# wgurecky/bipymc

Measured on AMD Instinct MI355X. Metric: chain-updates/sec, higher is better.
Workload: dtype f64

## Files before the change

bipymc_amd/csrc/kernels.h:

```cpp
#pragma once
#ifndef __HIPCC_RTC__
#include <hip/hip_runtime.h>
#include <stdint.h>
#endif

#include "philox.h"

#ifdef BPM_STAMPS
#define BPM_STAMP(i)                                                                          \
    do {                                                                                      \
        __builtin_amdgcn_sched_barrier(0);                                                    \
        unsigned long long _t;                                                                \
        asm volatile("s_memtime %0\n\ts_waitcnt lgkmcnt(0)" : "=s"(_t)::"memory");            \
        __builtin_amdgcn_sched_barrier(0);                                                    \
        bpm_stamp[i] = _t;                                                                    \
    } while (0)
#else
#define BPM_STAMP(i) do { } while (0)
#endif

#if defined(__HIP_DEVICE_COMPILE__) && !defined(__gfx942__) && !defined(__gfx950__)
#error "kernels.h: the ticket hand-overs rely on gfx942 / gfx950 memory behaviour (vmcnt counts stores; agent-scope atomics bypass the L2s): use __ATOMIC_RELEASE / __ATOMIC_ACQUIRE tickets on other targets"
#endif

// ... 119 lines not shown
    double* cr_part1;
    const double* cr_fold_part;
    const double* cr_fold_tot;
    double* cr_fold_out;
    uint32_t cr_fold_nb;
    uint32_t cr_chunk0, cr_n1;
    uint32_t adapt_on;
    uint32_t cr_gate;
    uint32_t hist_len;
    double gamma_scale, gamma_demc, epsilon, u_epsilon, p_snooker;
#ifdef BPM_LEAN_LAST
    uint32_t lean, pad_lean;
#endif
};

#ifdef BPM_TEST_HOOKS
__host__ __device__ __forceinline__ int32_t* trace_i32_of(const PhaseArgs& a) { return a.trace_i32; }
__host__ __device__ __forceinline__ double* trace_f64_of(const PhaseArgs& a) { return a.trace_f64; }
__host__ __device__ __forceinline__ uint8_t* trace_mask_of(const PhaseArgs& a) { return a.trace_mask; }
__host__ __device__ __forceinline__ void trace_set(PhaseArgs& a, int32_t* i, double* f, uint8_t* m) { a.trace_i32 = i; a.trace_f64 = f; a.trace_mask = m; }
#else
__host__ __device__ constexpr int32_t* trace_i32_of(const PhaseArgs&) { return nullptr; }
__host__ __device__ constexpr double* trace_f64_of(const PhaseArgs&) { return nullptr; }
__host__ __device__ constexpr uint8_t* trace_mask_of(const PhaseArgs&) { return nullptr; }
__host__ __device__ __forceinline__ void trace_set(PhaseArgs&, int32_t*, double*, uint8_t*) {}
#endif

template <int CTRL>
__device__ __forceinline__ double dpp_f64(double v) {
    const int lo = __builtin_amdgcn_update_dpp(0, __double2loint(v), CTRL, 0xF, 0xF, false);
    const int hi = __builtin_amdgcn_update_dpp(0, __double2hiint(v), CTRL, 0xF, 0xF, false);
    return __hiloint2double(hi, lo);
}
__device__ __forceinline__ double readlane_f64(double v, int lane) {
    return __hiloint2double(__builtin_amdgcn_readlane(__double2hiint(v), lane),
                            __builtin_amdgcn_readlane(__double2loint(v), lane));
}
template <int LPC>
__device__ __forceinline__ double gsum(double v) {
    static_assert(LPC == 1 || LPC == 4 || LPC == 16 || LPC == 32 || LPC == 64, "subgroup sizes");
    if (LPC >= 4) {
        v += dpp_f64<0xB1>(v);
        v += dpp_f64<0x4E>(v);
    }
    if (LPC >= 16) {
        v += dpp_f64<0x141>(v);
        v += dpp_f64<0x140>(v);
    }
    if (LPC == 32) v += __shfl_xor(v, 16);
    if (LPC == 64) v = (readlane_f64(v, 0) + readlane_f64(v, 16)) + (readlane_f64(v, 32) + readlane_f64(v, 48));
    return v;
}
template <int LPC>
__device__ __forceinline__ int gsum_i(int v) {
    if (LPC >= 4) {
        v += __builtin_amdgcn_update_dpp(0, v, 0xB1, 0xF, 0xF, false);
        v += __builtin_amdgcn_update_dpp(0, v, 0x4E, 0xF, 0xF, false);
    }
    if (LPC >= 16) {
        v += __builtin_amdgcn_update_dpp(0, v, 0x141, 0xF, 0xF, false);
        v += __builtin_amdgcn_update_dpp(0, v, 0x140, 0xF, 0xF, false);
    }
    if (LPC == 32) v += __shfl_xor(v, 16);
    if (LPC == 64)
        v = (__builtin_amdgcn_readlane(v, 0) + __builtin_amdgcn_readlane(v, 16)) +
            (__builtin_amdgcn_readlane(v, 32) + __builtin_amdgcn_readlane(v, 48));
    return v;
}

constexpr uint32_t CR_FINAL_MAX = 512;
__host__ __device__ inline uint32_t cr_chunks_of(uint32_t n_half, uint32_t g1) { return (n_half + g1 - 1u) / g1; }
struct CrTotals { double p[MAX_CR], d[MAX_CR], n[MAX_CR]; };
__device__ __forceinline__ void cr_finalize(bool any, uint32_t n_cr, CrTotals& T) {
    if (!any) return;
    uint32_t nz = 0;
#pragma unroll
    for (int m = 0; m < MAX_CR; ++m) nz += (m < (int)n_cr && T.n[m] != 0.0) ? 1u : 0u;
    if (nz == n_cr) {
#pragma unroll
        for (int m = 0; m < MAX_CR; ++m) if (m < (int)n_cr) T.p[m] = T.d[m] / T.n[m];
    }
    double sum = 0.0;
#pragma unroll
    for (int m = 0; m < MAX_CR; ++m) if (m < (int)n_cr) sum += T.p[m];
#pragma unroll
    for (int m = 0; m < MAX_CR; ++m) if (m < (int)n_cr) T.p[m] = T.p[m] / sum;
}
template <int ROUNDS>
__device__ __forceinline__ double cr_array_sum(const double* arr, uint32_t nb) {
    const uint32_t lane = threadIdx.x & (WAVE - 1);
    double v[ROUNDS];
#pragma unroll
    for (int r = 0; r < ROUNDS; ++r) {
        const uint32_t b = (uint32_t)r * WAVE + lane;
        const double x = arr[b < nb ? b : nb - 1u];
        v[r] = b < nb ? x : 0.0;
    }
    double s = 0.0;
#pragma unroll
    for (int r = 0; r < ROUNDS; ++r) s += v[r];
    return gsum<WAVE>(s);
}
template <int ROUNDS, bool PLAIN = false>
__device__ __forceinline__ void cr_fold(const double* tot, const double* part, uint32_t nb, uint32_t stride, uint32_t n_cr, CrTotals& T) {
    const uint32_t lane = threadIdx.x & (WAVE - 1);
#pragma unroll
// ... 30 lines not shown
                    if (tn > 0.0) { any = true; T.n[m0 + mm] += tn; T.d[m0 + mm] += td; }
                }
            }
        }
    }
    cr_finalize(any, n_cr, T);
}
__device__ __forceinline__ void cr_write_totals(const CrTotals& T, uint32_t n_cr, double* out) {
#pragma unroll
    for (int m = 0; m < MAX_CR; ++m)
        if (m < (int)n_cr) {
            __hip_atomic_store(&out[m], T.p[m], __ATOMIC_RELAXED, __HIP_MEMORY_SCOPE_AGENT);
            __hip_atomic_store(&out[MAX_CR + m], T.d[m], __ATOMIC_RELAXED, __HIP_MEMORY_SCOPE_AGENT);
            __hip_atomic_store(&out[2 * MAX_CR + m], T.n[m], __ATOMIC_RELAXED, __HIP_MEMORY_SCOPE_AGENT);
        }
}
__device__ __forceinline__ void cr_chunk_add(double& acc_d, double& acc_n, int m, int idx, double delta) {
    if (idx == m) { acc_d += delta; acc_n += 1.0; }
}

__device__ __forceinline__ double box_muller(uint32_t w1, uint32_t w2) {
    const double u1 = ((double)w1 + 1.0) * 2.3283064365386963e-10;
    const double u2 = u01_32(w2);
    return sqrt(-2.0 * log(u1)) * cos(6.283185307179586 * u2);
}

template <int TARGET, int LPC, int DPL>
struct Target;

template <int LPC, int DPL>
struct Target<TARGET_GAUSS, LPC, DPL> {
    struct Consts { double is[DPL]; double c0, a, b; };
    static __device__ __forceinline__ Consts load(int q, uint32_t dim, const double* tp) {
        Consts k;
        k.c0 = tp[1]; k.a = tp[2]; k.b = tp[3];
#pragma unroll
        for (int s = 0; s < DPL; ++s) {
            const uint32_t j = 2u * (uint32_t)(q + (s >> 1) * LPC) + (s & 1);
            k.is[s] = j < dim ? tp[4 + j] : 0.0;
        }
        return k;
    }
    static __device__ __forceinline__ double eval(const double* v, int q, uint32_t dim, const Consts& k) {
        double s1 = 0.0, s2 = 0.0;
#pragma unroll
        for (int s = 0; s < DPL; ++s) {
            const uint32_t j = 2u * (uint32_t)(q + (s >> 1) * LPC) + (s & 1);
            if (j < dim) {
                const double z = v[s] * k.is[s];
                s1 += z;
                s2 += z * z;
            }
        }
        s1 = gsum<LPC>(s1);
        s2 = gsum<LPC>(s2);
        return k.c0 - 0.5 * (k.a * s2 - k.b * s1 * s1);
    }
};

template <int LPC, int DPL>
struct Target<TARGET_MIXTURE, LPC, DPL> {
    struct Consts { double p[16]; };
    static __device__ __forceinline__ Consts load(int, uint32_t, const double* tp) {
        Consts k;
#pragma unroll
        for (int i = 0; i < 16; ++i) k.p[i] = tp[i];
        return k;
    }
    static __device__ __forceinline__ double eval(const double* v, int q, uint32_t dim, const Consts& k) {
        double q0 = 0.0, q1 = 0.0;
#pragma unroll
        for (int u = 0; u < DPL / 2; ++u) {
            const uint32_t j = 2u * (uint32_t)(q + u * LPC);
            if (j + 1 < dim) {
#pragma unroll
                for (int c = 0; c < 2; ++c) {
                    const double* p = k.p + 2 + 7 * c;
                    const double a = (v[2 * u] - p[0]) * p[2];
                    const double b = (v[2 * u + 1] - p[1]) * p[3];
                    const double qq = (a * a - 2.0 * p[4] * a * b + b * b) * p[5];
                    if (c == 0) q0 += qq; else q1 += qq;
                }
            }
        }
        q0 = gsum<LPC>(q0);
        q1 = gsum<LPC>(q1);
        const double npairs = (double)(dim / 2);
        const double c0 = k.p[0] + npairs * k.p[8] - 0.5 * q0;
        const double c1 = k.p[1] + npairs * k.p[15] - 0.5 * q1;
        const double m = fmax(c0, c1);
        return m + log(exp(c0 - m) + exp(c1 - m));
    }
};

template <int LPC, int DPL>
struct Target<TARGET_BANANA, LPC, DPL> {
    struct Consts { double p[9]; };
    static __device__ __forceinline__ Consts load(int, uint32_t, const double* tp) {
        Consts k;
#pragma unroll
        for (int i = 0; i < 9; ++i) k.p[i] = tp[i];
        return k;
    }
    static __device__ __forceinline__ double eval(const double* v, int, uint32_t, const Consts& k) {
        const double a = k.p[7], b = k.p[8];
        const double x1 = v[0] / a;
        const double x2 = (v[1] - b * (x1 * x1 + a * a)) * a;
        const double u = (x1 - k.p[0]) * k.p[2];
        const double w = (x2 - k.p[1]) * k.p[3];
        return k.p[6] - 0.5 * (u * u - 2.0 * k.p[4] * u * w + w * w) * k.p[5];
    }
};

template <int DPL>
struct Work {
    double x[DPL];
    double p[DPL];
    double delta;
    double log_corr;
    double gamma;
    uint32_t acc_hi, acc_lo;
    uint32_t item;
    uint32_t pos_own;
    double ll_cur;
    uint32_t acc_prev;
    double w_mean[DPL], w_m2[DPL];
    int cr_idx, d_prime, jump, snk;
    uint32_t maskbits;
};

typedef double bpm_d2v __attribute__((ext_vector_type(2)));
template <int LPC, int DPL>
__device__ __forceinline__ void load_row(const double* row, int q, uint32_t ld, double* v) {
#pragma unroll
    for (int u = 0; u < DPL / 2; ++u) {
        const uint32_t pi = (uint32_t)(q + u * LPC);
        double2 t = make_double2(0.0, 0.0);
        if (2 * pi < ld) t = reinterpret_cast<const double2*>(row)[pi];
        v[2 * u] = t.x;
        v[2 * u + 1] = t.y;
    }
}
template <int LPC, int DPL>
__device__ __forceinline__ void store_row(double* row, int q, uint32_t ld, const double* v) {
#pragma unroll
    for (int u = 0; u < DPL / 2; ++u) {
        const uint32_t pi = (uint32_t)(q + u * LPC);
        if (2 * pi < ld) reinterpret_cast<double2*>(row)[pi] = make_double2(v[2 * u], v[2 * u + 1]);
    }
}

template <int LPC, int DPL>
__device__ __forceinline__ void store_row_wt(double* row, int q, uint32_t ld, const double* v) {
#pragma unroll
    for (int u = 0; u < DPL / 2; ++u) {
        const uint32_t pi = (uint32_t)(q + u * LPC);
        if (2 * pi < ld) {
            __hip_atomic_store(row + 2 * pi, v[2 * u], __ATOMIC_RELAXED, __HIP_MEMORY_SCOPE_AGENT);
            __hip_atomic_store(row + 2 * pi + 1, v[2 * u + 1], __ATOMIC_RELAXED, __HIP_MEMORY_SCOPE_AGENT);
        }
    }
}

template <int LPC, int DPL>
__device__ __forceinline__ void store_row_wt16(double* row, int q, uint32_t ld, const double* v) {
#pragma unroll
    for (int u = 0; u < DPL / 2; ++u) {
        const uint32_t pi = (uint32_t)(q + u * LPC);
        if (2 * pi < ld) {
            bpm_d2v t = {v[2 * u], v[2 * u + 1]};
            bpm_d2v* p = reinterpret_cast<bpm_d2v*>(row) + pi;
            asm volatile("global_store_dwordx4 %0, %1, off sc1" ::"v"(p), "v"(t) : "memory");
        }
    }
}

template <int LPC, int DPL>
__device__ __forceinline__ void store_row_sys(double* row, int q, uint32_t ld, const double* v) {
#pragma unroll
    for (int u = 0; u < DPL / 2; ++u) {
        const uint32_t pi = (uint32_t)(q + u * LPC);
        if (2 * pi < ld) {
            __hip_atomic_store(row + 2 * pi, v[2 * u], __ATOMIC_RELAXED, __HIP_MEMORY_SCOPE_SYSTEM);
            __hip_atomic_store(row + 2 * pi + 1, v[2 * u + 1], __ATOMIC_RELAXED, __HIP_MEMORY_SCOPE_SYSTEM);
// ... 139 lines not shown
        const uint32_t uq = (uint32_t)q, hdr_lane = npairs + 2u * (uint32_t)NP;
        const uint32_t pidx = uq - npairs;
        const uint32_t slot = uq < npairs ? SLOT_DIM0 + uq : (uq < hdr_lane ? SLOT_PAIR0 + (pidx >> 2) : SLOT_HDR0);
        const u32x4 wb = chain_block(a.seed, c, a.t, slot);
        wpair[0] = wb;
        h0.x = (uint32_t)__builtin_amdgcn_readlane((int)wb.x, hdr_lane);
        h0.y = (uint32_t)__builtin_amdgcn_readlane((int)wb.y, hdr_lane);
        h0.z = (uint32_t)__builtin_amdgcn_readlane((int)wb.z, hdr_lane);
        h0.w = (uint32_t)__builtin_amdgcn_readlane((int)wb.w, hdr_lane);
        BPM_STAMP(2);
        uint32_t mine = 0;
        if (uq >= npairs && uq < hdr_lane) {
            const uint32_t p = pidx >> 1;
            uint32_t ia, ib;
            distinct_pair((p & 1) ? wb.z : wb.x, (p & 1) ? wb.w : wb.y, a.M, ia, ib);
            uint32_t pos = (pidx & 1) ? ib : ia;
            if (a.mode == 2) pos += (pos >= c) ? 1u : 0u;
            mine = pos_to_chain(a, a.pool_off + pos);
        }
#pragma unroll
        for (int i = 0; i < 2 * NP; ++i) part.r[i] = (uint32_t)__builtin_amdgcn_readlane((int)mine, npairs + i);
    } else if (QUAD) {
        wpair[0] = chain_block(a.seed, c, a.t, SLOT_DIM0 + (uint32_t)q);
        const u32x4 wb = chain_block(a.seed, c, a.t, q == 1 ? SLOT_PAIR0 : (q == 2 ? SLOT_PAIR0 + 1u : SLOT_HDR0));
        h0.x = quad_bcast<0>(wb.x); h0.y = quad_bcast<0>(wb.y); h0.z = quad_bcast<0>(wb.z); h0.w = quad_bcast<0>(wb.w);
        uint32_t i0 = 0, i1 = 0, i2 = 0, i3 = 0;
        if (q == 1 || q == 2) {
            uint32_t ia, ib;
            distinct_pair(wb.x, wb.y, a.M, ia, ib);
            i0 = pos_to_chain(a, a.pool_off + ia); i1 = pos_to_chain(a, a.pool_off + ib);
            if (q == 1) {
                distinct_pair(wb.z, wb.w, a.M, ia, ib);
                i2 = pos_to_chain(a, a.pool_off + ia); i3 = pos_to_chain(a, a.pool_off + ib);
            }
        }
        part.r[0] = quad_bcast<1>(i0); part.r[1] = quad_bcast<1>(i1); part.r[2] = quad_bcast<1>(i2); part.r[3] = quad_bcast<1>(i3);
        part.r[4] = quad_bcast<2>(i0); part.r[5] = quad_bcast<2>(i1);
    } else {
        h0 = chain_block(a.seed, c, a.t, SLOT_HDR0);
#pragma unroll
        for (int u = 0; u < DPL / 2; ++u) wpair[u] = chain_block(a.seed, c, a.t, SLOT_DIM0 + (uint32_t)(q + u * LPC));
        if (FAST) {
#pragma unroll
            for (int i = 0; i < 2 * NP; ++i) part.r[i] = pos_to_chain(a, a.pool_off + partner_pos(a, c, (uint32_t)i, 2u * NP));
        }
        if (RL) {
            uint32_t mine = 0;
            if (q < 2 * NP) mine = pos_to_chain(a, a.pool_off + partner_pos(a, c, (uint32_t)q, 2u * NP));
#pragma unroll
            for (int i = 0; i < 2 * NP; ++i) part.r[i] = (uint32_t)__builtin_amdgcn_readlane((int)mine, i);
        }
    }
    BPM_STAMP(3);
    wk.acc_hi = h0.z; wk.acc_lo = h0.w;
    const double u_sel = (double)(h0.x >> 16) * 1.52587890625e-05;
    const double u_gam = (double)(h0.x & 0xFFFFu) * 1.52587890625e-05;
    uint32_t snk_id[3] = {0u, 0u, 0u};
    if (SNK_DIRECT && snk_possible && planned) {
        snk_id[0] = rec[5 + 2 * P]; snk_id[1] = rec[6 + 2 * P]; snk_id[2] = rec[7 + 2 * P];
    } else if (SNK_DIRECT && snk_possible && (u_sel < a.p_snooker || trace_i32_of(a) != nullptr)) {
        const u32x4 ws = chain_block(a.seed, c, a.t, SLOT_SNK);
        uint32_t iz, i1, i2;
        distinct_three(ws.x, ws.y, ws.z, a.M, iz, i1, i2);
        snk_id[0] = pos_to_chain(a, a.pool_off + iz);
        snk_id[1] = pos_to_chain(a, a.pool_off + i1);
        snk_id[2] = pos_to_chain(a, a.pool_off + i2);
    }
    if (!REGS || (snk_possible && !SNK_DIRECT)) {
#pragma unroll 1
        for (uint32_t idx = (uint32_t)q; idx < npart; idx += LPC)
            s_part[cw * MAX_PARTNERS + idx] = planned ? rec[5 + idx] : pos_to_chain(a, a.pool_off + partner_pos(a, c, idx, 2 * P));
        __builtin_amdgcn_fence(__ATOMIC_RELEASE, "wavefront");
        __builtin_amdgcn_wave_barrier();
        __builtin_amdgcn_fence(__ATOMIC_ACQUIRE, "wavefront");
    }

    constexpr int NPX = NP > 0 ? NP : 1;
    double ra[NPX][DPL], rb[NPX][DPL];
    if (DREAM && NP > 0) {
#pragma unroll
        for (int p = 0; p < NP; ++p) {
            load_row<LPC, DPL>(row_ptr(a.L, part.get(2 * p)), q, ld, ra[p]);
            load_row<LPC, DPL>(row_ptr(a.L, part.get(2 * p + 1)), q, ld, rb[p]);
        }
    }
    BPM_STAMP(7);
    if (dims_late) wpair[0] = chain_block(a.seed, c, a.t, SLOT_DIM0 + (uint32_t)q);
    if (DREAM) early(wk);

    double eps_n[DPL], eps_u[DPL];
    uint32_t maskbits = 0;
    wk.cr_idx = -1; wk.d_prime = (int)dim; wk.jump = 0; wk.snk = 0; wk.delta = 0.0; wk.log_corr = 0.0;
    uint32_t thr = 65536u;
    if (DREAM) {
        const double uc = u_sel;
        double cum = 0.0;
        int idx = (int)a.n_cr - 1;
        bool found = false;
#pragma unroll
        for (int m = 0; m < MAX_CR; ++m) {
            if (m < (int)a.n_cr) {
                cum += pcr[m];
                if (!found && uc < cum) { idx = m; thr = a.thr[m]; found = true; }
            }
        }
        if (!found) {
#pragma unroll
            for (int m = 0; m < MAX_CR; ++m) if (m == (int)a.n_cr - 1) thr = a.thr[m];
        }
        wk.cr_idx = idx;
    }
    int cnt = 0;
#pragma unroll
    for (int u = 0; u < DPL / 2; ++u) {
        const uint32_t pi = (uint32_t)(q + u * LPC);
        const uint32_t j0 = 2u * pi;
        eps_n[2 * u] = 0.0; eps_n[2 * u + 1] = 0.0; eps_u[2 * u] = 0.0; eps_u[2 * u + 1] = 0.0;
        if (j0 < dim) {
            const u32x4 wj = wpair[u];
            const bool two = j0 + 1 < dim;
            if (a.epsilon > 0.0) {
                double n0, n1;
                box_muller_pair_f32(wj.z, wj.w, n0, n1);
                eps_n[2 * u] = a.epsilon * n0;
                if (two) eps_n[2 * u + 1] = a.epsilon * n1;
            }
            if (DREAM) {
                if (a.u_epsilon > 0.0) {
                    eps_u[2 * u] = -a.u_epsilon + (2.0 * a.u_epsilon) * (((double)(wj.y >> 16) + 0.5) * 1.52587890625e-05);
                    if (two) eps_u[2 * u + 1] = -a.u_epsilon + (2.0 * a.u_epsilon) * (((double)(wj.y & 0xFFFFu) + 0.5) * 1.52587890625e-05);
                }
                if ((wj.x >> 16) <= thr) { maskbits |= 1u << (2 * u); ++cnt; }
                if (two && (wj.x & 0xFFFFu) <= thr) { maskbits |= 1u << (2 * u + 1); ++cnt; }
            }
        }
    }
    if (DREAM) {
        if (LPC == WAVE) {
            cnt = 0;
#pragma unroll
            for (int sb = 0; sb < DPL; ++sb) cnt += (int)__popcll(__ballot((maskbits >> sb) & 1u));
        } else {
            cnt = gsum_i<LPC>(cnt);
        }
        if (cnt == 0) {
            const uint32_t f = mulhi32(h0.y, dim);
#pragma unroll
            for (int s = 0; s < DPL; ++s) {
                const uint32_t j = 2u * (uint32_t)(q + (s >> 1) * LPC) + (s & 1);
                if (j == f) maskbits |= 1u << s;
            }
            cnt = 1;
        }
        wk.d_prime = cnt;
    }
    wk.maskbits = maskbits;

    if (DREAM) {
        double gamma;
        if (LPC == WAVE && (uint32_t)cnt < (uint32_t)(WAVE * DPL)) {
            double gsel = gtab[0];
#pragma unroll
            for (int u = 1; u < DPL; ++u) gsel = ((cnt >> 6) == u) ? gtab[u] : gsel;
            gamma = readlane_f64(gsel, cnt & 63);
        } else if (LPC * DPL < WAVE) {
            gamma = __shfl(gt_lane, cnt);
        } else {
            gamma = a.gamma_tab[cnt];
        }
        if (a.k % 5 == 0 && !(u_gam < 0.2)) { gamma = 1.0; wk.jump = 1; }
        wk.gamma = gamma;
        double sum[DPL];
        if (NP > 0) {
#pragma unroll
            for (int s = 0; s < DPL; ++s) {
                sum[s] = ra[0][s] - rb[0][s];
#pragma unroll
                for (int p = 1; p < NP; ++p) sum[s] = sum[s] + (ra[p][s] - rb[p][s]);
            }
        } else {
#pragma unroll
            for (int s = 0; s < DPL; ++s) sum[s] = 0.0;
#pragma unroll 1
            for (uint32_t p = 0; p < P; ++p) {
                double ra[DPL], rb[DPL];
                load_row<LPC, DPL>(row_ptr(a.L, part.lds[2 * p]), q, ld, ra);
                load_row<LPC, DPL>(row_ptr(a.L, part.lds[2 * p + 1]), q, ld, rb);
#pragma unroll
                for (int s = 0; s < DPL; ++s) sum[s] = (p == 0) ? (ra[s] - rb[s]) : (sum[s] + (ra[s] - rb[s]));
            }
        }
#pragma unroll
        for (int s = 0; s < DPL; ++s) {
            const double jump = (1.0 + eps_u[s]) * gamma * sum[s] + eps_n[s];
            wk.p[s] = ((maskbits >> s) & 1u) ? (jump + wk.x[s]) : wk.x[s];
        }
        BPM_STAMP(4);
        if (a.adapt_on && a.cr_gate) {
            const double* m2 = wk.w_m2;
            double dl = 0.0;
#pragma unroll
            for (int s = 0; s < DPL; ++s) {
                const uint32_t j = 2u * (uint32_t)(q + (s >> 1) * LPC) + (s & 1);
                if (j < dim) {
                    const double df = wk.x[s] - wk.p[s];
                    dl += m2[s] > 0.0 ? (df * df * (double)a.hist_len) / m2[s] : (df * df) / 1e-24;
                }
            }
            wk.delta = gsum<LPC>(dl);
        }
    } else {
        double gamma = a.gamma_demc;
        if (a.mode != 2 && a.k % 10 == 0 && !(u_gam < 0.1)) { gamma = 1.0; wk.jump = 1; }
        wk.gamma = gamma;
        double ra[DPL], rb[DPL];
        const bool ids_in_regs = REGS && (!snk_possible || SNK_DIRECT);
        const uint32_t ca = ids_in_regs ? part.get(0) : part.lds[0];
        const uint32_t cb = ids_in_regs ? part.get(1) : part.lds[1];
        const bool do_snk = snk_possible && u_sel < a.p_snooker;
        if (LPC == 1) asm volatile("" ::"v"(ca), "v"(cb), "v"(snk_id[0]), "v"(snk_id[1]), "v"(snk_id[2]));
        load_row<LPC, DPL>(row_ptr(a.L, ca), q, ld, ra);
        load_row<LPC, DPL>(row_ptr(a.L, cb), q, ld, rb);
        double rz[DPL], r1[DPL], r2[DPL];
#pragma unroll
// ... 28 lines not shown
                for (int s = 0; s < DPL; ++s) {
                    const uint32_t j = 2u * (uint32_t)(q + (s >> 1) * LPC) + (s & 1);
                    const double df = wk.x[s] - rz[s];
                    double pv = wk.x[s] + gs * df;
                    pv = pv + eps_n[s];
                    if (j >= dim) pv = wk.x[s];
                    wk.p[s] = pv;
                    const double dn = pv - rz[s];
                    n2p += dn * dn;
                }
                n2p = gsum<LPC>(n2p);
                wk.log_corr = 0.5 * (double)(dim - 1) * (log(n2p) - log(n2));
                wk.snk = 1;
            }
        }
    }
    if (trace_i32_of(a) && active) {
        if (q == 0) {
            int32_t* tr = trace_i32_of(a) + (uint64_t)(c - a.lo) * TRACE_I32;
            tr[0] = wk.cr_idx; tr[1] = wk.d_prime; tr[2] = wk.jump; tr[4] = wk.snk;
            if (REGS) {
#pragma unroll
                for (int i = 0; i < 2 * NP; ++i) tr[5 + i] = (int32_t)part.get(i);
            }
            const bool regs = REGS && (!snk_possible || SNK_DIRECT);
#pragma unroll 1
            for (uint32_t i = regs ? 2u * P : 0u; i < MAX_PARTNERS; ++i) {
                int32_t v = -1;
                const uint32_t ks = i - 2u * P;
                if (i < npart) v = regs ? (int32_t)(ks == 1u ? snk_id[1] : (ks == 2u ? snk_id[2] : snk_id[0])) : (int32_t)part.lds[i];
                tr[5 + i] = v;
            }
        }
        if (trace_mask_of(a)) {
#pragma unroll
            for (int s = 0; s < DPL; ++s) {
                const uint32_t j = 2u * (uint32_t)(q + (s >> 1) * LPC) + (s & 1);
                if (j < dim) trace_mask_of(a)[(uint64_t)(c - a.lo) * dim + j] = (uint8_t)((maskbits >> s) & 1u);
            }
        }
    }
}

template <int ALGO, int LPC, int DPL, int LEAN = 0 , bool CRP_W = false>
__device__ __forceinline__ void finish_update(const PhaseArgs& a, uint32_t c, bool active, int q,
                                              const Work<DPL>& wk, double ll_prop) {
    const uint32_t ld = a.L.ld;
    const uint32_t li = c - a.lo;
    const double ll_cur = wk.ll_cur;
    double alpha = exp((ll_prop + wk.log_corr) - ll_cur);
    const bool is_nan = alpha != alpha;
    alpha = fmin(1.0, alpha);
    alpha = fmax(0.0, alpha);
    const bool accepted = !is_nan && (u01_53(wk.acc_hi, wk.acc_lo) < alpha);
    const bool lean = LEAN == 2 || (LEAN == 1 && a.lean != 0u);
    if (lean) {
        const unsigned long long m = __ballot(active && accepted && q == 0);
        if ((threadIdx.x & (WAVE - 1)) == 0 && m != 0ull)
            __hip_atomic_fetch_add(&a.acc_count[a.L.n_local + ((blockIdx.x * (blockDim.x / WAVE) + (threadIdx.x / WAVE)) & (ACC_SHARDS - 1))],
                                   (uint32_t)__popcll(m), __ATOMIC_RELAXED, __HIP_MEMORY_SCOPE_AGENT);
    }
    if (!active) return;
    if (q == 0) {
        if (accepted && !lean) {
#if defined(BPM_TEST_HOOKS) && defined(BPM_FAKE_NO_LL)
            if (LPC < WAVE) {} else
#endif
            if (LPC < WAVE) __hip_atomic_fetch_add(&a.acc_count[li], 1u, __ATOMIC_RELAXED, __HIP_MEMORY_SCOPE_AGENT);
            else if (a.wt) __hip_atomic_store(&a.acc_count[li], wk.acc_prev + 1u, __ATOMIC_RELAXED, __HIP_MEMORY_SCOPE_AGENT);
            else a.acc_count[li] = wk.acc_prev + 1u;
        }
        if (is_nan) atomicAdd(&a.counters[2], 1ull);
        if (a.accbits) a.accbits[a.acc_by_item ? wk.item : li] = accepted ? (uint8_t)1 : (uint8_t)0;
    }
    double nv[DPL];
#pragma unroll
    for (int s = 0; s < DPL; ++s) nv[s] = accepted ? wk.p[s] : wk.x[s];
    const double new_ll = accepted ? ll_prop : ll_cur;
    if (a.x_next) {
        store_row<LPC, DPL>(a.x_next + (uint32_t)(li * ld), q, ld, nv);
        if (accepted && q == 0 && !lean) a.ll[li] = new_ll;
    } else if (accepted) {
        if (a.wt == 2u) {
            store_row_wt16<LPC, DPL>(row_ptr(a.L, c), q, ld, nv);
#if defined(BPM_TEST_HOOKS) && defined(BPM_FAKE_NO_LL)
            if (LPC < WAVE) {} else
#endif
            if (q == 0 && !lean) __hip_atomic_store(&a.ll[li], new_ll, __ATOMIC_RELAXED, __HIP_MEMORY_SCOPE_AGENT);
        } else if (a.wt) {
            store_row_wt<LPC, DPL>(row_ptr(a.L, c), q, ld, nv);
            if (q == 0 && !lean) __hip_atomic_store(&a.ll[li], new_ll, __ATOMIC_RELAXED, __HIP_MEMORY_SCOPE_AGENT);
        } else {
            store_row<LPC, DPL>(row_ptr(a.L, c), q, ld, nv);
            if (q == 0 && !lean) a.ll[li] = new_ll;
        }
    }
    if (a.pack && accepted) {
        double* sub = a.pack + (uint32_t)((li & (a.pack_nsub - 1u)) * a.pack_stride);
        uint32_t slot = 0;
        if (q == 0) slot = atomicAdd(reinterpret_cast<uint32_t*>(sub), 1u);
        slot = __shfl(slot, (threadIdx.x & (WAVE - 1)) - q);
        if (slot < a.pack_cap) {
            if (q == 0) sub[2 + slot] = (double)c;
            store_row<LPC, DPL>(sub + 2 + a.pack_cap + (uint32_t)(slot * ld), q, ld, nv);
        }
    }
    if (a.n_peers) {
        const uint32_t row_off = (uint32_t)(row_ptr(a.L, c) - a.L.G);
        const bool slots = ALGO == ALGO_DREAM && a.adapt_on && a.cr_gate && q == 0;
        const uint32_t d_off = (uint32_t)(delta_ptr(a.L, c) - a.L.G), c_off = (uint32_t)(cridx_ptr(a.L, c) - a.L.G);
        const bool gated = a.adapt_on && a.cr_gate;
#pragma unroll 1
        for (uint32_t p = 0; p < a.n_peers; ++p) {
            double* pg = reinterpret_cast<double*>(a.peer_tab[p]);
            if (accepted) store_row_sys<LPC, DPL>(pg + row_off, q, ld, nv);
            if (slots) {
                __hip_atomic_store(pg + d_off, gated ? wk.delta : 0.0, __ATOMIC_RELAXED, __HIP_MEMORY_SCOPE_SYSTEM);
                __hip_atomic_store(pg + c_off, gated ? (double)wk.cr_idx : -1.0, __ATOMIC_RELAXED, __HIP_MEMORY_SCOPE_SYSTEM);
            }
        }
    }
    const uint32_t hi = a.hist_by_pos ? wk.pos_own : li;
    if (a.hist_row) store_row_stream<LPC, DPL>(a.hist_row + (uint32_t)(hi * ld), q, ld, nv);
    if (a.llhist_row && q == 0) {
        double* dst_ll = &a.llhist_row[a.hist_by_pos == 1u ? wk.pos_own : li];
        if (LPC < WAVE) __builtin_nontemporal_store(new_ll, dst_ll); else *dst_ll = new_ll;
    }
    if (ALGO == ALGO_DREAM) {
        if (a.adapt_on) {
            double mean[DPL], m2[DPL];
#pragma unroll
            for (int s = 0; s < DPL; ++s) { mean[s] = wk.w_mean[s]; m2[s] = wk.w_m2[s]; }
            const double cntp = (double)(a.hist_len + 1);
#pragma unroll
            for (int s = 0; s < DPL; ++s) {
                const double d1 = nv[s] - mean[s];
                mean[s] = mean[s] + d1 / cntp;
                m2[s] = m2[s] + d1 * (nv[s] - mean[s]);
            }
            if (a.wt) {
                store_row_wt16<LPC, DPL>(a.w_mean + (uint32_t)(li * 2u * ld), q, ld, mean);
                store_row_wt16<LPC, DPL>(a.w_m2 + (uint32_t)(li * 2u * ld), q, ld, m2);
            } else {
                store_row_stream<LPC, DPL>(a.w_mean + (uint32_t)(li * 2u * ld), q, ld, mean);
                store_row_stream<LPC, DPL>(a.w_m2 + (uint32_t)(li * 2u * ld), q, ld, m2);
            }
        }
        if (q == 0 && a.adapt_on && !(CRP_W && a.cr_part1 != nullptr)) {
            const bool gated = a.adapt_on && a.cr_gate;
            if (a.wt) {
                __hip_atomic_store(delta_ptr(a.L, c), gated ? wk.delta : 0.0, __ATOMIC_RELAXED, __HIP_MEMORY_SCOPE_AGENT);
                __hip_atomic_store(cridx_ptr(a.L, c), gated ? (double)wk.cr_idx : -1.0, __ATOMIC_RELAXED, __HIP_MEMORY_SCOPE_AGENT);
            } else {
                *delta_ptr(a.L, c) = gated ? wk.delta : 0.0;
                *cridx_ptr(a.L, c) = gated ? (double)wk.cr_idx : -1.0;
            }
        }
    }
    if (trace_i32_of(a) && q == 0) {
        trace_i32_of(a)[(uint64_t)li * TRACE_I32 + 3] = accepted ? 1 : 0;
        double* tf = trace_f64_of(a) + (uint64_t)li * TRACE_F64;
        tf[0] = alpha; tf[1] = ll_prop; tf[2] = wk.delta; tf[3] = wk.gamma;
    }
    if (a.n_peers) asm volatile("s_waitcnt vmcnt(0)" ::: "memory");
}

template <int LPC>
__device__ __forceinline__ void pin_args(const PhaseArgs& a) {
    if (LPC != WAVE) {
        asm volatile("" ::"s"(a.L.G), "s"(a.L.ld), "s"(a.L.dim), "s"(a.ll), "s"(a.hist_row), "s"(a.llhist_row), "s"(a.tparams),
                     "s"(a.cr_state), "s"(a.acc_count), "s"(a.perm_tab), "s"(a.inv_tab), "s"(a.gamma_tab), "s"(a.plan), "s"(a.pack),
                     "s"(a.thr[0]), "s"(a.thr[1]), "s"(a.thr[2]), "s"(a.seed), "s"(a.t), "s"(a.k), "s"(a.N),
                     "s"(a.lo), "s"(a.upd_off), "s"(a.n_upd), "s"(a.pool_off), "s"(a.M), "s"(a.mode), "s"(a.n_items), "s"(a.n_cr));
        asm volatile("" ::"s"(a.adapt_on), "s"(a.cr_gate), "s"(a.hist_len), "s"(a.epsilon), "s"(a.u_epsilon), "s"(a.L.n_local),
                     "s"(a.L.world), "s"(a.L.magic), "s"(a.counters), "s"(a.pack_cap), "s"(a.pack_nsub), "s"(a.pack_stride));
    }
}

__device__ __forceinline__ bool resolve_chain(const PhaseArgs& a, uint32_t w, uint32_t& c) {
    bool active = w < a.n_items;
    if (a.mode == 0) {
        c = own_pos_to_chain(a, a.upd_off + (active ? w : 0u));
    } else if (a.mode == 2) {
        c = a.lo + (active ? w : 0u);
    } else {
        c = a.lo + (active ? w : 0u);
        const uint32_t pos = chain_to_pos(a, c);
        active = active && (pos - a.upd_off) < a.n_upd;
    }
    return active;
}

__host__ inline bool phase_args_hot_sharded(const PhaseArgs& a, bool dream, bool with_plan) {
    return a.mode == 0 && (a.rec_tab != nullptr) == with_plan && trace_i32_of(a) == nullptr && a.pack == nullptr && a.x_next == nullptr &&
           a.adapt_on == 0 && a.epsilon > 0.0 && a.L.world > 1 &&
           a.perm_tab != nullptr && a.inv_tab != nullptr && a.stamps == nullptr && (a.accbits != nullptr || a.n_peers > 0) && a.replay == 0 &&
           (!dream || (a.u_epsilon > 0.0 && a.n_cr == 3));
}
__host__ inline bool phase_args_hot(const PhaseArgs& a, bool dream, bool with_plan, bool adapting) {
    return a.n_peers == 0 && a.mode == 0 && (a.rec_tab != nullptr) == with_plan && trace_i32_of(a) == nullptr && a.pack == nullptr && a.x_next == nullptr &&
           (a.adapt_on != 0) == adapting && a.epsilon > 0.0 && a.L.world == 1 &&
           a.perm_tab != nullptr && a.inv_tab != nullptr && a.lo == 0 && a.stamps == nullptr && a.accbits == nullptr && a.replay == 0 &&
           (!dream || (a.u_epsilon > 0.0 && a.n_cr == 3));
}
template <int ALGO, int TARGET, int LPC, int DPL, int NP, int HOT = 0>
__global__ __launch_bounds__(block_for_hot(LPC, HOT, DPL)) void phase_fused_kernel(
#ifdef BPM_PRELOAD
    const uint32_t* pl_plan, uint32_t pl_upd_off, uint32_t pl_n_items, uint32_t pl_mode,
#endif
    const PhaseArgs a_in) {
    constexpr bool COPY = (HOT != 0);
    constexpr bool SHARD = (HOT == 5 || HOT == 6), ADAPT = (HOT == 3 || HOT == 4), NOPLAN = (HOT == 2 || HOT == 4 || HOT == 6);
    PhaseArgs a_hot;
    if (COPY) {
        a_hot = a_in;
        a_hot.mode = 0u; trace_set(a_hot, nullptr, nullptr, nullptr); a_hot.pack = nullptr;
        a_hot.replay = 0u; a_hot.x_next = nullptr; a_hot.adapt_on = ADAPT ? 1u : 0u; a_hot.stamps = nullptr;
        if (!ADAPT) a_hot.cr_fold_part = nullptr;
        if (!SHARD) { a_hot.accbits = nullptr; a_hot.lo = 0; a_hot.L.world = 1; a_hot.acc_by_item = 0u; a_hot.n_peers = 0u; a_hot.peer_tab = nullptr; }
        if (ALGO == ALGO_DREAM) a_hot.n_cr = 3;
        if (NOPLAN) { a_hot.plan = nullptr; a_hot.rec_tab = nullptr; }
    }
    const PhaseArgs& a = COPY ? a_hot : a_in;
    if (HOT) {
        __builtin_assume(a_in.mode == 0u); __builtin_assume(a_in.pack == nullptr);
#ifdef BPM_TEST_HOOKS
        __builtin_assume(a_in.trace_i32 == nullptr);
#endif
        __builtin_assume(a_in.x_next == nullptr); __builtin_assume(a_in.adapt_on == (ADAPT ? 1u : 0u)); __builtin_assume(a_in.stamps == nullptr);
        if (!SHARD) { __builtin_assume(a_in.lo == 0); __builtin_assume(a_in.L.world == 1); }
        __builtin_assume(a_in.epsilon > 0.0);
        __builtin_assume(a_in.perm_tab != nullptr); __builtin_assume(a_in.inv_tab != nullptr);
        if (ALGO == ALGO_DREAM) { __builtin_assume(a_in.u_epsilon > 0.0); __builtin_assume(a_in.n_cr == 3); }
    }
#ifdef BPM_PRELOAD
    if (HOT) { __builtin_assume(pl_mode == 0u); __builtin_assume((pl_plan != nullptr) == !NOPLAN); }
#else
    const uint32_t* pl_plan = a.rec_tab;
    const uint32_t pl_upd_off = a.rec_off, pl_n_items = a.n_items, pl_mode = a.mode;
#endif
    constexpr int BLK = block_for_hot(LPC, HOT, DPL);
    constexpr bool CRP = ALGO == ALGO_DREAM && hot_is_adapt(HOT) && crp_shape(LPC, DPL);
    __shared__ uint32_t s_part[(BLK / LPC) * MAX_PARTNERS];
    const int lane = threadIdx.x;
    const int cw = lane / LPC, q = lane % LPC;
    const uint32_t w = blockIdx.x * (BLK / LPC) + cw;
#ifdef BPM_STAMPS
    unsigned long long bpm_stamp[8] = {0, 0, 0, 0, 0, 0, 0, 0};
    unsigned long long bpm_rt0;
    asm volatile("s_memrealtime %0\n\ts_waitcnt lgkmcnt(0)" : "=s"(bpm_rt0)::"memory");
    BPM_STAMP(0);
#endif
    pin_args<LPC>(a);
    uint32_t c;
    bool active;
    const uint32_t* rec = nullptr;
    bool run = true;
    double cr_d = 0.0;
    int cr_i = -1;
    if (LPC == WAVE && pl_plan && !(CRP && w >= pl_n_items)) {
        active = w < pl_n_items;
        if (!active) return;
        uint32_t pos;
        if (pl_mode == 0) {
            pos = pl_upd_off + w;
        } else {
            pos = a.inv_tab[a.lo + w];
            if ((pos - pl_upd_off) >= a.n_upd) return;
        }
        pos = __builtin_amdgcn_readfirstlane(pos);
        rec = pl_plan + (uint32_t)(pos * PLAN_WORDS);
        c = rec[0];
    } else {
        active = resolve_chain(a, w, c);
    }
    if (LPC == WAVE && !active) {
        if (CRP) run = false; else return;
    }
    PcrGiven pcr_fold;
    if constexpr (CRP) {
        pcr_fold.on = a.cr_fold_part != nullptr;
        if (pcr_fold.on) {
            __shared__ double s_tot[2 * MAX_CR];
            constexpr uint32_t NWV = (uint32_t)(BLK / WAVE);
            const uint32_t n_cr = a.n_cr, wv = (uint32_t)lane / (uint32_t)WAVE;
            for (uint32_t k = wv; k < 2u * n_cr; k += NWV) {
                const uint32_t arr = k < n_cr ? k : (uint32_t)MAX_CR + (k - n_cr);
                const double tsum = cr_array_sum<CR_FINAL_MAX / WAVE>(a.cr_fold_part + (uint64_t)arr * a.cr_fold_nb, a.cr_fold_nb);
                if ((lane & (WAVE - 1)) == 0) s_tot[arr] = tsum;
            }
            __syncthreads();
            CrTotals T;
#pragma unroll
            for (int m = 0; m < MAX_CR; ++m) { T.p[m] = a.cr_fold_tot[m]; T.d[m] = a.cr_fold_tot[MAX_CR + m]; T.n[m] = a.cr_fold_tot[2 * MAX_CR + m]; }
            bool any = false;
#pragma unroll
            for (int m = 0; m < MAX_CR; ++m) {
                if (m < (int)n_cr) {
                    const double td = s_tot[m], tn = s_tot[MAX_CR + m];
                    if (tn > 0.0) { any = true; T.n[m] += tn; T.d[m] += td; }
                }
            }
            cr_finalize(any, n_cr, T);
            if (blockIdx.x == 0 && lane == 0) cr_write_totals(T, n_cr, a.cr_fold_out);
#pragma unroll
            for (int m = 0; m < MAX_CR; ++m)
                pcr_fold.p[m] = __hiloint2double(__builtin_amdgcn_readfirstlane(__double2hiint(T.p[m])), __builtin_amdgcn_readfirstlane(__double2loint(T.p[m])));
        }
    }
  if (run) {
    if (LPC == WAVE) c = __builtin_amdgcn_readfirstlane(c);
    const typename Target<TARGET, LPC, DPL>::Consts tc = Target<TARGET, LPC, DPL>::load(q, a.L.dim, a.tparams);
    Work<DPL> wk;
    wk.item = w;
    wk.pos_own = a.upd_off + (active ? w : 0u);
    constexpr bool LEAN = lean_scalars<TARGET, LPC>();
    const uint32_t dim_early = a.L.dim;
    constexpr bool LEAN_CT = LEAN && lean_always<TARGET>();
#ifdef BPM_STAMPS
    bpm_stamp[1] = 0; BPM_STAMP(1);
    unsigned long long* const stamp_arg = bpm_stamp;
#else
    unsigned long long* const stamp_arg = nullptr;
#endif
    if constexpr (LEAN) {
        const bool lean_early = LEAN_CT || a.lean != 0u;
        auto early = [tc, q, dim_early, lean_early](Work<DPL>& k) { if (lean_early) k.ll_cur = Target<TARGET, LPC, DPL>::eval(k.x, q, dim_early, tc); };
        make_proposal<ALGO, LPC, DPL, NP, (LEAN_CT ? 0 : 2)>(a, c, active, q, cw, s_part, wk, rec, stamp_arg, early, pcr_fold);
    } else if constexpr (CRP) {
        make_proposal<ALGO, LPC, DPL, NP>(a, c, active, q, cw, s_part, wk, rec, stamp_arg, NoEarly(), pcr_fold);
    } else {
        make_proposal<ALGO, LPC, DPL, NP>(a, c, active, q, cw, s_part, wk, rec, stamp_arg);
    }
    const double ll_prop = Target<TARGET, LPC, DPL>::eval(wk.p, q, a.L.dim, tc);
    BPM_STAMP(5);
    finish_update<ALGO, LPC, DPL, (LEAN_CT ? 2 : (LEAN ? 1 : 0)), CRP>(a, c, active, q, wk, ll_prop);
    if (CRP && active && a.adapt_on && a.cr_gate) { cr_d = wk.delta; cr_i = wk.cr_idx; }
    BPM_STAMP(6);
#ifdef BPM_STAMPS
    if (bpm_stamp[2] == 0) bpm_stamp[2] = bpm_rt0;
    {
        unsigned long long rt;
        asm volatile("s_memrealtime %0\n\ts_waitcnt lgkmcnt(0)" : "=s"(rt)::"memory");
        bpm_stamp[7] = (rt & 0x0FFFFFFFFFFFFFFFull) | ((unsigned long long)(__builtin_amdgcn_s_getreg((31 << 11) | 20) & 0xF) << 60);
    }
    if (a.stamps && lane == 0) for (int i = 0; i < 8; ++i) a.stamps[(uint64_t)w * 8 + i] = bpm_stamp[i];
#endif
  }
    if (CRP && a.cr_part1) {
        constexpr int G1 = cr_g1(LPC);
        if (LPC == WAVE) {
            __shared__ double s_crd[G1];
            __shared__ int s_cri[G1];
            if (q == 0) { s_crd[cw] = cr_d; s_cri[cw] = cr_i; }
            __syncthreads();
            if (cw == 0 && q < (int)a.n_cr) {
                double sd = 0.0, sn = 0.0;
#pragma unroll
                for (int k = 0; k < G1; ++k) cr_chunk_add(sd, sn, q, s_cri[k], s_crd[k]);
                const uint32_t ch = a.cr_chunk0 + blockIdx.x;
                __hip_atomic_store(&a.cr_part1[(uint64_t)q * a.cr_n1 + ch], sd, __ATOMIC_RELAXED, __HIP_MEMORY_SCOPE_AGENT);
                __hip_atomic_store(&a.cr_part1[(uint64_t)(MAX_CR + q) * a.cr_n1 + ch], sn, __ATOMIC_RELAXED, __HIP_MEMORY_SCOPE_AGENT);
            }
        } else {
            const int wl = lane & (WAVE - 1);
            double sd = 0.0, sn = 0.0;
#pragma unroll
            for (int k = 0; k < G1; ++k) {
                const double dk = readlane_f64(cr_d, k * LPC);
                const int ik = __builtin_amdgcn_readlane(cr_i, k * LPC);
                cr_chunk_add(sd, sn, wl, ik, dk);
            }
            const uint32_t ch = a.cr_chunk0 + (blockIdx.x * (BLK / WAVE) + (uint32_t)(lane / WAVE));
            if (wl < (int)a.n_cr && (ch - a.cr_chunk0) * (uint32_t)G1 < a.n_items) {
                __hip_atomic_store(&a.cr_part1[(uint64_t)wl * a.cr_n1 + ch], sd, __ATOMIC_RELAXED, __HIP_MEMORY_SCOPE_AGENT);
                __hip_atomic_store(&a.cr_part1[(uint64_t)(MAX_CR + wl) * a.cr_n1 + ch], sn, __ATOMIC_RELAXED, __HIP_MEMORY_SCOPE_AGENT);
            }
        }
    }
}

#ifdef BPM_EXPERIMENT_XCD
__device__ __forceinline__ unsigned long long xcd_now() {
    unsigned long long t;
    asm volatile("s_memrealtime %0\n\ts_waitcnt lgkmcnt(0)" : "=s"(t)::"memory");
    return t;
}
__device__ __forceinline__ uint32_t xcd_l2_add(uint32_t* p, uint32_t v) {
    uint32_t old;
    asm volatile("global_atomic_add %0, %1, %2, off sc0\n\ts_waitcnt vmcnt(0)" : "=v"(old) : "v"(p), "v"(v) : "memory");
    return old;
}
__device__ __forceinline__ bool xcd_barrier(uint32_t* ctl, uint32_t target, unsigned long long deadline) {
// ... 149 lines not shown
    c = (uint32_t)__builtin_amdgcn_readfirstlane((int)c);
    Work<DPL> wk;
    make_proposal<ALGO, LPC, DPL, NP>(a, c, true, lane, wv, s_part, wk, rec);
    store_row<LPC, DPL>(row_ptr(a.L, c), lane, a.L.ld, wk.p);
}

template <int ALGO, int LPC, int DPL, int NP = 0>
__global__ __launch_bounds__(block_for(LPC)) void phase_propose_kernel(const PhaseArgs a) {
    __shared__ uint32_t s_part[(block_for(LPC) / LPC) * MAX_PARTNERS];
    const int lane = threadIdx.x;
    const int cw = lane / LPC, q = lane % LPC;
    const uint32_t w = blockIdx.x * (block_for(LPC) / LPC) + cw;
    uint32_t c;
    const bool active = resolve_chain(a, w, c);
    if (w < a.n_items && q == 0) a.ids_buf[w] = active ? (int32_t)c : -1;
    if (LPC == WAVE && !active) return;
    if (LPC == WAVE) c = __builtin_amdgcn_readfirstlane(c);
    Work<DPL> wk;
    make_proposal<ALGO, LPC, DPL, NP>(a, c, active, q, cw, s_part, wk);
    if (!active) return;
    store_row<LPC, DPL>(a.prop_buf + (uint64_t)w * a.L.ld, q, a.L.ld, wk.p);
    if (q == 0) {
        a.aux_buf[w] = wk.log_corr;
        if (ALGO == ALGO_DREAM) {
            const bool gated = a.adapt_on && a.cr_gate;
            *delta_ptr(a.L, c) = gated ? wk.delta : 0.0;
            *cridx_ptr(a.L, c) = gated ? (double)wk.cr_idx : -1.0;
        }
    }
}

template <int ALGO, int LPC, int DPL>
__global__ __launch_bounds__(block_for(LPC)) void phase_commit_kernel(const PhaseArgs a) {
    const int lane = threadIdx.x;
    const int cw = lane / LPC, q = lane % LPC;
    const uint32_t w = blockIdx.x * (block_for(LPC) / LPC) + cw;
    bool active = w < a.n_items;
    int32_t id = active ? a.ids_buf[w] : -1;
    active = active && id >= 0;
    if (LPC == WAVE && !active) return;
    const uint32_t c = active ? (uint32_t)id : a.lo;
    Work<DPL> wk;
    load_row<LPC, DPL>(row_ptr(a.L, c), q, a.L.ld, wk.x);
    load_row<LPC, DPL>(a.prop_buf + (uint64_t)(active ? w : 0u) * a.L.ld, q, a.L.ld, wk.p);
    wk.log_corr = active ? a.aux_buf[w] : 0.0;
    wk.ll_cur = a.ll[c - a.lo];
    wk.acc_prev = a.acc_count[c - a.lo];
    if (ALGO == ALGO_DREAM && a.adapt_on) {
        load_row<LPC, DPL>(a.w_mean + (uint32_t)((c - a.lo) * 2u * a.L.ld), q, a.L.ld, wk.w_mean);
        load_row<LPC, DPL>(a.w_m2 + (uint32_t)((c - a.lo) * 2u * a.L.ld), q, a.L.ld, wk.w_m2);
    }
    const double ll_prop = active ? a.aux_buf[a.L.n_local + w] : 0.0;
    const u32x4 h0 = chain_block(a.seed, c, a.t, SLOT_HDR0);
    wk.acc_hi = h0.z; wk.acc_lo = h0.w;
    wk.delta = 0.0; wk.gamma = 0.0; wk.cr_idx = -1; wk.d_prime = 0; wk.jump = 0; wk.snk = 0; wk.maskbits = 0; wk.item = w; wk.pos_own = 0u;
    if (ALGO == ALGO_DREAM && active) {
        wk.delta = *delta_ptr(a.L, c);
        wk.cr_idx = (int)*cridx_ptr(a.L, c);
    }
    PhaseArgs b = a;
    if (ALGO == ALGO_DREAM) b.cr_gate = (wk.cr_idx >= 0) ? 1u : 0u;
    finish_update<ALGO, LPC, DPL>(b, c, active, q, wk, ll_prop);
}

constexpr int CR_L1_THREADS = 256;
template <int G1, int J>
__device__ __forceinline__ int cr_bcast_i(int v) {
    if (G1 == 4) return __builtin_amdgcn_update_dpp(0, v, J * 0x55, 0xF, 0xF, false);
    if (G1 == 16) return __builtin_amdgcn_update_dpp(0, v, 0x150 + J, 0xF, 0xF, false);
    return __builtin_amdgcn_readlane(v, J);
}
template <int G1, int J>
__device__ __forceinline__ void cr_l1_steps(int idx, double dl, int m0, double& sd0, double& sn0, double& sd1, double& sn1) {
    const int ij = cr_bcast_i<G1, J>(idx);
    const double dj = __hiloint2double(cr_bcast_i<G1, J>(__double2hiint(dl)), cr_bcast_i<G1, J>(__double2loint(dl)));
    cr_chunk_add(sd0, sn0, m0, ij, dj);
    if (G1 == 4) cr_chunk_add(sd1, sn1, m0 + 4, ij, dj);
    if constexpr (J + 1 < G1) cr_l1_steps<G1, J + 1>(idx, dl, m0, sd0, sn0, sd1, sn1);
}
template <int G1>
__global__ __launch_bounds__(CR_L1_THREADS) void cr_level1_kernel(Layout L, PermKey pk, const uint32_t* perm_tab, uint32_t N, uint32_t n_cr, uint32_t n1, double* part1) {
    const uint32_t t = blockIdx.x * CR_L1_THREADS + threadIdx.x;
    const uint32_t ch = t / G1, k = t % G1;
    const uint32_t n_first = (N + 1u) / 2u, c_first = cr_chunks_of(n_first, G1);
    const bool second = ch >= c_first;
    const uint32_t pos = second ? n_first + (ch - c_first) * G1 + k : ch * G1 + k;
    const bool valid = ch < n1 && pos < (second ? N : n_first);
    int idx = -1;
    double dl = 0.0;
    if (valid) {
        const uint32_t c = perm_tab ? perm_tab[pos] : perm_fwd(pos, pk);
        idx = (int)*cridx_ptr(L, c);
        dl = *delta_ptr(L, c);
    }
    static_assert(MAX_CR <= 8, "a chunk's lanes cover the CR values: lane k sums value k (and k + 4 when G1 == 4)");
    double sd0 = 0.0, sn0 = 0.0, sd1 = 0.0, sn1 = 0.0;
    cr_l1_steps<G1, 0>(idx, dl, (int)k, sd0, sn0, sd1, sn1);
    if (ch < n1) {
        if (k < n_cr) {
            __hip_atomic_store(&part1[(uint64_t)k * n1 + ch], sd0, __ATOMIC_RELAXED, __HIP_MEMORY_SCOPE_AGENT);
            __hip_atomic_store(&part1[(uint64_t)(MAX_CR + k) * n1 + ch], sn0, __ATOMIC_RELAXED, __HIP_MEMORY_SCOPE_AGENT);
        }
        if (G1 == 4 && k + 4u < n_cr) {
            __hip_atomic_store(&part1[(uint64_t)(k + 4u) * n1 + ch], sd1, __ATOMIC_RELAXED, __HIP_MEMORY_SCOPE_AGENT);
            __hip_atomic_store(&part1[(uint64_t)(MAX_CR + k + 4u) * n1 + ch], sn1, __ATOMIC_RELAXED, __HIP_MEMORY_SCOPE_AGENT);
        }
    }
// ... 735 lines not shown
```

Baseline: 772.9 million.

## Interleave dual reductions, scalarize wave-uniform values, hoist history store, unmasked row loads

```diff
diff --git a/bipymc_amd/csrc/kernels.h b/bipymc_amd/csrc/kernels.h
--- a/bipymc_amd/csrc/kernels.h
+++ b/bipymc_amd/csrc/kernels.h
@@ -195,6 +195,28 @@
     return v;
 }
 template <int LPC>
+__device__ __forceinline__ void gsum2(double& v, double& w) {
+    static_assert(LPC == 1 || LPC == 4 || LPC == 16 || LPC == 32 || LPC == 64, "subgroup sizes");
+    if (LPC >= 4) {
+        const double v1 = dpp_f64<0xB1>(v), w1 = dpp_f64<0xB1>(w);
+        v += v1; w += w1;
+        const double v2 = dpp_f64<0x4E>(v), w2 = dpp_f64<0x4E>(w);
+        v += v2; w += w2;
+    }
+    if (LPC >= 16) {
+        const double v3 = dpp_f64<0x141>(v), w3 = dpp_f64<0x141>(w);
+        v += v3; w += w3;
+        const double v4 = dpp_f64<0x140>(v), w4 = dpp_f64<0x140>(w);
+        v += v4; w += w4;
+    }
+    if (LPC == 32) { const double vs = __shfl_xor(v, 16), ws = __shfl_xor(w, 16); v += vs; w += ws; }
+    if (LPC == 64) {
+        const double va = readlane_f64(v, 0) + readlane_f64(v, 16), wa = readlane_f64(w, 0) + readlane_f64(w, 16);
+        const double vb = readlane_f64(v, 32) + readlane_f64(v, 48), wb = readlane_f64(w, 32) + readlane_f64(w, 48);
+        v = va + vb; w = wa + wb;
+    }
+}
+template <int LPC>
 __device__ __forceinline__ int gsum_i(int v) {
     if (LPC >= 4) {
         v += __builtin_amdgcn_update_dpp(0, v, 0xB1, 0xF, 0xF, false);
@@ -331,8 +353,7 @@
                 s2 += z * z;
             }
         }
-        s1 = gsum<LPC>(s1);
-        s2 = gsum<LPC>(s2);
+        gsum2<LPC>(s1, s2);
         return k.c0 - 0.5 * (k.a * s2 - k.b * s1 * s1);
     }
 };
@@ -398,7 +419,7 @@
     double delta;
     double log_corr;
     double gamma;
-    uint32_t acc_hi, acc_lo;
+    double u_acc;
     uint32_t item;
     uint32_t pos_own;
     double ll_cur;
@@ -409,6 +430,17 @@
 };
 
 typedef double bpm_d2v __attribute__((ext_vector_type(2)));
+template <int LPC, int DPL>
+__device__ __forceinline__ void load_row_all(const double* row, int q, uint32_t ld, double* v) {
+    const uint32_t last = (ld >> 1) - 1u;
+#pragma unroll
+    for (int u = 0; u < DPL / 2; ++u) {
+        const uint32_t pi = (uint32_t)(q + u * LPC);
+        const double2 t = reinterpret_cast<const double2*>(row)[pi < last ? pi : last];
+        v[2 * u] = t.x;
+        v[2 * u + 1] = t.y;
+    }
+}
 template <int LPC, int DPL>
 __device__ __forceinline__ void load_row(const double* row, int q, uint32_t ld, double* v) {
 #pragma unroll
@@ -654,7 +686,7 @@
         }
     }
     BPM_STAMP(3);
-    wk.acc_hi = h0.z; wk.acc_lo = h0.w;
+    wk.u_acc = u01_53(h0.z, h0.w);
     const double u_sel = (double)(h0.x >> 16) * 1.52587890625e-05;
     const double u_gam = (double)(h0.x & 0xFFFFu) * 1.52587890625e-05;
     uint32_t snk_id[3] = {0u, 0u, 0u};
@@ -682,8 +714,13 @@
     if (DREAM && NP > 0) {
 #pragma unroll
         for (int p = 0; p < NP; ++p) {
-            load_row<LPC, DPL>(row_ptr(a.L, part.get(2 * p)), q, ld, ra[p]);
-            load_row<LPC, DPL>(row_ptr(a.L, part.get(2 * p + 1)), q, ld, rb[p]);
+            if (LPC == WAVE) {
+                load_row_all<LPC, DPL>(row_ptr(a.L, part.get(2 * p)), q, ld, ra[p]);
+                load_row_all<LPC, DPL>(row_ptr(a.L, part.get(2 * p + 1)), q, ld, rb[p]);
+            } else {
+                load_row<LPC, DPL>(row_ptr(a.L, part.get(2 * p)), q, ld, ra[p]);
+                load_row<LPC, DPL>(row_ptr(a.L, part.get(2 * p + 1)), q, ld, rb[p]);
+            }
         }
     }
     BPM_STAMP(7);
@@ -772,6 +809,12 @@
         }
         if (a.k % 5 == 0 && !(u_gam < 0.2)) { gamma = 1.0; wk.jump = 1; }
         wk.gamma = gamma;
+        if (LPC == WAVE) {
+            int u_hi = __builtin_amdgcn_readfirstlane(__double2hiint(wk.u_acc)), u_lo = __builtin_amdgcn_readfirstlane(__double2loint(wk.u_acc));
+            asm volatile("" : "+s"(u_hi), "+s"(u_lo));
+            wk.u_acc = __hiloint2double(u_hi, u_lo);
+            asm volatile("" ::"s"(a.wt), "s"(a.hist_by_pos), "s"(a.upd_off), "s"(a.hist_row), "s"(a.llhist_row), "s"(a.ll), "s"(a.acc_count));
+        }
         double sum[DPL];
         if (NP > 0) {
 #pragma unroll
@@ -906,7 +949,7 @@
     const bool is_nan = alpha != alpha;
     alpha = fmin(1.0, alpha);
     alpha = fmax(0.0, alpha);
-    const bool accepted = !is_nan && (u01_53(wk.acc_hi, wk.acc_lo) < alpha);
+    const bool accepted = !is_nan && (wk.u_acc < alpha);
     const bool lean = LEAN == 2 || (LEAN == 1 && a.lean != 0u);
     if (lean) {
         const unsigned long long m = __ballot(active && accepted && q == 0);
@@ -915,6 +958,12 @@
                                    (uint32_t)__popcll(m), __ATOMIC_RELAXED, __HIP_MEMORY_SCOPE_AGENT);
     }
     if (!active) return;
+    double nv[DPL];
+#pragma unroll
+    for (int s = 0; s < DPL; ++s) nv[s] = accepted ? wk.p[s] : wk.x[s];
+    const double new_ll = accepted ? ll_prop : ll_cur;
+    const uint32_t hi = a.hist_by_pos ? wk.pos_own : li;
+    if (LPC == WAVE && a.hist_row) store_row_stream<LPC, DPL>(a.hist_row + (uint32_t)(hi * ld), q, ld, nv);
     if (q == 0) {
         if (accepted && !lean) {
 #if defined(BPM_TEST_HOOKS) && defined(BPM_FAKE_NO_LL)
@@ -927,10 +976,6 @@
         if (is_nan) atomicAdd(&a.counters[2], 1ull);
         if (a.accbits) a.accbits[a.acc_by_item ? wk.item : li] = accepted ? (uint8_t)1 : (uint8_t)0;
     }
-    double nv[DPL];
-#pragma unroll
-    for (int s = 0; s < DPL; ++s) nv[s] = accepted ? wk.p[s] : wk.x[s];
-    const double new_ll = accepted ? ll_prop : ll_cur;
     if (a.x_next) {
         store_row<LPC, DPL>(a.x_next + (uint32_t)(li * ld), q, ld, nv);
         if (accepted && q == 0 && !lean) a.ll[li] = new_ll;
@@ -974,8 +1019,7 @@
             }
         }
     }
-    const uint32_t hi = a.hist_by_pos ? wk.pos_own : li;
-    if (a.hist_row) store_row_stream<LPC, DPL>(a.hist_row + (uint32_t)(hi * ld), q, ld, nv);
+    if (LPC != WAVE && a.hist_row) store_row_stream<LPC, DPL>(a.hist_row + (uint32_t)(hi * ld), q, ld, nv);
     if (a.llhist_row && q == 0) {
         double* dst_ll = &a.llhist_row[a.hist_by_pos == 1u ? wk.pos_own : li];
         if (LPC < WAVE) __builtin_nontemporal_store(new_ll, dst_ll); else *dst_ll = new_ll;
@@ -1045,6 +1089,11 @@
     return active;
 }
 
+#ifdef BPM_STAMPS
+__host__ inline bool stamps_allow_hot(const PhaseArgs&) { return true; }
+#else
+__host__ inline bool stamps_allow_hot(const PhaseArgs& a) { return a.stamps == nullptr; }
+#endif
 __host__ inline bool phase_args_hot_sharded(const PhaseArgs& a, bool dream, bool with_plan) {
     return a.mode == 0 && (a.rec_tab != nullptr) == with_plan && trace_i32_of(a) == nullptr && a.pack == nullptr && a.x_next == nullptr &&
            a.adapt_on == 0 && a.epsilon > 0.0 && a.L.world > 1 &&
@@ -1054,7 +1103,7 @@
 __host__ inline bool phase_args_hot(const PhaseArgs& a, bool dream, bool with_plan, bool adapting) {
     return a.n_peers == 0 && a.mode == 0 && (a.rec_tab != nullptr) == with_plan && trace_i32_of(a) == nullptr && a.pack == nullptr && a.x_next == nullptr &&
            (a.adapt_on != 0) == adapting && a.epsilon > 0.0 && a.L.world == 1 &&
-           a.perm_tab != nullptr && a.inv_tab != nullptr && a.lo == 0 && a.stamps == nullptr && a.accbits == nullptr && a.replay == 0 &&
+           a.perm_tab != nullptr && a.inv_tab != nullptr && a.lo == 0 && stamps_allow_hot(a) && a.accbits == nullptr && a.replay == 0 &&
            (!dream || (a.u_epsilon > 0.0 && a.n_cr == 3));
 }
 template <int ALGO, int TARGET, int LPC, int DPL, int NP, int HOT = 0>
@@ -1069,7 +1118,12 @@
     if (COPY) {
         a_hot = a_in;
         a_hot.mode = 0u; trace_set(a_hot, nullptr, nullptr, nullptr); a_hot.pack = nullptr;
-        a_hot.replay = 0u; a_hot.x_next = nullptr; a_hot.adapt_on = ADAPT ? 1u : 0u; a_hot.stamps = nullptr;
+        a_hot.replay = 0u; a_hot.x_next = nullptr; a_hot.adapt_on = ADAPT ? 1u : 0u;
+#ifndef BPM_STAMPS
+        a_hot.stamps = nullptr;
+#else
+        if (SHARD) a_hot.stamps = nullptr;
+#endif
         if (!ADAPT) a_hot.cr_fold_part = nullptr;
         if (!SHARD) { a_hot.accbits = nullptr; a_hot.lo = 0; a_hot.L.world = 1; a_hot.acc_by_item = 0u; a_hot.n_peers = 0u; a_hot.peer_tab = nullptr; }
         if (ALGO == ALGO_DREAM) a_hot.n_cr = 3;
@@ -1081,7 +1135,10 @@
 #ifdef BPM_TEST_HOOKS
         __builtin_assume(a_in.trace_i32 == nullptr);
 #endif
-        __builtin_assume(a_in.x_next == nullptr); __builtin_assume(a_in.adapt_on == (ADAPT ? 1u : 0u)); __builtin_assume(a_in.stamps == nullptr);
+        __builtin_assume(a_in.x_next == nullptr); __builtin_assume(a_in.adapt_on == (ADAPT ? 1u : 0u));
+#ifndef BPM_STAMPS
+        __builtin_assume(a_in.stamps == nullptr);
+#endif
         if (!SHARD) { __builtin_assume(a_in.lo == 0); __builtin_assume(a_in.L.world == 1); }
         __builtin_assume(a_in.epsilon > 0.0);
         __builtin_assume(a_in.perm_tab != nullptr); __builtin_assume(a_in.inv_tab != nullptr);
@@ -1168,6 +1225,7 @@
     Work<DPL> wk;
     wk.item = w;
     wk.pos_own = a.upd_off + (active ? w : 0u);
+    if (LPC == WAVE) wk.pos_own = (uint32_t)__builtin_amdgcn_readfirstlane((int)wk.pos_own);
     constexpr bool LEAN = lean_scalars<TARGET, LPC>();
     const uint32_t dim_early = a.L.dim;
     constexpr bool LEAN_CT = LEAN && lean_always<TARGET>();
@@ -1192,7 +1250,7 @@
     if (CRP && active && a.adapt_on && a.cr_gate) { cr_d = wk.delta; cr_i = wk.cr_idx; }
     BPM_STAMP(6);
 #ifdef BPM_STAMPS
-    if (bpm_stamp[2] == 0) bpm_stamp[2] = bpm_rt0;
+    if (bpm_stamp[2] == 0) { bpm_stamp[2] = bpm_rt0; bpm_stamp[1] = bpm_stamp[7]; }
     {
         unsigned long long rt;
         asm volatile("s_memrealtime %0\n\ts_waitcnt lgkmcnt(0)" : "=s"(rt)::"memory");
@@ -1448,7 +1506,7 @@
     }
     const double ll_prop = active ? a.aux_buf[a.L.n_local + w] : 0.0;
     const u32x4 h0 = chain_block(a.seed, c, a.t, SLOT_HDR0);
-    wk.acc_hi = h0.z; wk.acc_lo = h0.w;
+    wk.u_acc = u01_53(h0.z, h0.w);
     wk.delta = 0.0; wk.gamma = 0.0; wk.cr_idx = -1; wk.d_prime = 0; wk.jump = 0; wk.snk = 0; wk.maskbits = 0; wk.item = w; wk.pos_own = 0u;
     if (ALGO == ALGO_DREAM && active) {
         wk.delta = *delta_ptr(a.L, c);
```

Measured after the change: 781.7 million (median of 6 runs). 1.1% higher.
